# volivan239/raytracing-course-hw

Hardware: AMD Instinct MI355X
Metric: Msamples/sec at 1920x1080x256spp (higher is better)
Workload: dtype f32; 1 GPU; synth_room_v1_1920x1080x256; scene=synth_room_v1 (seed 20241223), triangles=268816, emissive_triangles=4204, width=1920, height=1080, spp=256, ray_depth=6, parallelism=pixel tiles 32x32 round-robin over 1 GPU(s), bvh_nodes=265605, bvh_depth=24, light_bvh_depth=19, device_bytes=120573816

## Files before the change

raytracing-course-hw_amd/csrc/device/rt_device.h:

```cpp
#pragma once
#include <hip/hip_runtime.h>
#include "rt_types.h"

#define RT_DEV __device__ __forceinline__

namespace rtamd {
namespace dev {

struct F3 { float x, y, z; };
RT_DEV F3 f3(float x, float y, float z) { F3 r; r.x = x; r.y = y; r.z = z; return r; }
RT_DEV F3 f3(const float *p) { return f3(p[0], p[1], p[2]); }
RT_DEV F3 operator+(F3 a, F3 b) { return f3(a.x + b.x, a.y + b.y, a.z + b.z); }
RT_DEV F3 operator-(F3 a, F3 b) { return f3(a.x - b.x, a.y - b.y, a.z - b.z); }
RT_DEV F3 operator*(F3 a, F3 b) { return f3(a.x * b.x, a.y * b.y, a.z * b.z); }
RT_DEV F3 operator*(float k, F3 p) { return f3(k * p.x, k * p.y, k * p.z); }
RT_DEV F3 neg(F3 a) { return f3(-a.x, -a.y, -a.z); }
RT_DEV float dot(F3 a, F3 b) { return a.x * b.x + a.y * b.y + a.z * b.z; }
RT_DEV F3 crossr(F3 a, F3 o) { return f3(a.z * o.y - a.y * o.z, a.x * o.z - a.z * o.x, a.y * o.x - a.x * o.y); }
RT_DEV float len2(F3 a) { return dot(a, a); }
RT_DEV float len(F3 a) { return sqrtf(len2(a)); }
RT_DEV F3 normalize(F3 a) { return (1.0f / len(a)) * a; }
RT_DEV float smin(float a, float b) { return (b < a) ? b : a; }
RT_DEV float smax(float a, float b) { return (a < b) ? b : a; }

// ... 193 lines not shown
    float yy = (c1 * T.a2 - c2 * T.a1) / T.den;
    float xx = T.a2 == 0 ? (c1 - T.b1 * yy) / T.a1 : (c2 - T.b2 * yy) / T.a2;
    u = xx; v = yy;
    if (u < 0 || v < 0 || u + v > 1) return false;
    return true;
}

RT_DEV bool tri_test_closer(const TriIsect &T, F3 o, F3 d, float keep_t, float &t, float &u, float &v, bool &inside) {
    F3 a = f3(T.ax, T.ay, T.az), n = f3(T.nx, T.ny, T.nz);
    F3 ro = o - a;
    float dn = dot(d, n);
    t = -dot(ro, n) / dn;
    if (!(t > 0 && t < RT_T_MAX)) return false;
    if (t > keep_t) return false;
    inside = dn > 0;
    F3 p = ro + t * d;
    float c1 = RT_MAGIC1_0 * p.x + RT_MAGIC1_1 * p.y + RT_MAGIC1_2 * p.z;
    float c2 = RT_MAGIC2_0 * p.x + RT_MAGIC2_1 * p.y + RT_MAGIC2_2 * p.z;
    float yy = (c1 * T.a2 - c2 * T.a1) / T.den;
    float xx = T.a2 == 0 ? (c1 - T.b1 * yy) / T.a1 : (c2 - T.b2 * yy) / T.a2;
    u = xx; v = yy;
    if (u < 0 || v < 0 || u + v > 1) return false;
    return true;
}

RT_DEV TriIsect load_isect(const TriIsect *p) {
    const float4 *q = reinterpret_cast<const float4 *>(p);
    float4 a = q[0], b = q[1], c = q[2];
    TriIsect T;
    T.ax = a.x; T.ay = a.y; T.az = a.z; T.nx = a.w;
    T.ny = b.x; T.nz = b.y; T.a1 = b.z; T.b1 = b.w;
    T.a2 = c.x; T.b2 = c.y; T.den = c.z; T.pad = __float_as_uint(c.w);
    return T;
}

struct RayInv { F3 o, inv; };
RT_DEV RayInv make_ray_inv(F3 o, F3 d) {
    RayInv r;
    r.o = o;
    float dx = fabsf(d.x) > 1e-30f ? d.x : copysignf(1e-30f, d.x);
    float dy = fabsf(d.y) > 1e-30f ? d.y : copysignf(1e-30f, d.y);
    float dz = fabsf(d.z) > 1e-30f ? d.z : copysignf(1e-30f, d.z);
    r.inv = f3(1.0f / dx, 1.0f / dy, 1.0f / dz);
    return r;
}
RT_DEV bool slab_test(float4 lo, float4 hi, const RayInv &r, float tbest, float &tnear) {
// ... 425 lines not shown
```

raytracing-course-hw_amd/csrc/device/rt_exact.h:

```cpp
#pragma once
#include "rt_kernels_hw8.h"

namespace rtamd {
namespace dev {

#define PT_SHADE_EXACT 4
#define WF_MISS 0xFFFFFFFFu
#define WF_INSIDE_BIT 0x40000000u
#define WF_GAP_SHIFT 24
#define WF_INDEX_MASK 0x00FFFFFFu
#define WF_SAMPLE_MASK 0x01FFFFFFu
#define WF_VERIFIED_BIT 0x80000000u

RT_DEV bool ref_box_test(F3 mn, F3 mx, F3 o, F3 d, float &t, bool &inside) {
    const F3 s = 0.5f * (mx - mn);
    const F3 oc = o - 0.5f * (mn + mx);
    const F3 a = neg(s) - oc, b = s - oc;
    const float a1x = a.x / d.x, a1y = a.y / d.y, a1z = a.z / d.z;
    const float a2x = b.x / d.x, a2y = b.y / d.y, a2z = b.z / d.z;
    const float t1x = smin(a1x, a2x), t2x = smax(a1x, a2x);
    const float t1y = smin(a1y, a2y), t2y = smax(a1y, a2y);
    const float t1z = smin(a1z, a2z), t2z = smax(a1z, a2z);
    const float t1 = smax(smax(t1x, t1y), t1z);
    const float t2 = smin(smin(t2x, t2y), t2z);
// ... 140 lines not shown
                const float4 mlo = rec[2 * m];
                if (slab_test(mlo, rec[2 * m + 1], r, RT_T_MAX, tn)) {
                    const uint32_t fi = __float_as_uint(mlo.w);
                    const TriIsect T = load_isect(S.tri_isect + fi);
                    float t, u, v; bool inside;
                    if (tri_test(T, o, d, t, u, v, inside)) {
                        const float4 *bx = reinterpret_cast<const float4 *>(S.tri_box) + 2 * (size_t)fi;
                        const float4 blo = bx[0], bhi = bx[1];
                        if (!pt_deep_inside(f3(blo.x, blo.y, blo.z), f3(bhi.x, bhi.y, bhi.z), o + t * d, d, t, S.box_c2)) pierced = true;
                    }
                }
            }
        }
    }
    return pierced;
}

RT_DEV bool pt_light_test(const LightRec *L, F3 x, F3 d, bool &last, uint32_t &index, float &t, float &u, float &v, bool &inside) {
    const TriIsect T = load_isect(&L->isect);
    last = (T.pad & 1u) != 0;
    index = T.pad >> 1;
    return tri_test(T, x, d, t, u, v, inside);
}
RT_DEV float pt_light_pdf_hit(const SceneView &S, const LightRec *L, F3 x, F3 d, float t, float u, float v, bool inside, bool &robust) {
    robust = true;
    const float4 *q = reinterpret_cast<const float4 *>(L) + 3;
    float4 q1 = q[1], q2 = q[2], q3 = q[3];
    float point_prob = q1.z;
    F3 n3 = f3(q1.w, q2.x, q2.y), dn1 = f3(q2.z, q2.w, q3.x), dn2 = f3(q3.y, q3.z, q3.w);
    F3 sn = n3 + u * dn1 + v * dn2;
    sn = normalize(sn);
    if (inside) sn = neg(sn);
    if (S.hw7) { const TriIsect T = load_isect(&L->isect); F3 n = f3(T.nx, T.ny, T.nz); sn = normalize(inside ? neg(n) : n); }
    F3 y = x + t * d;
    if (S.exact_boxes == 1u) {
        const float4 blo = q[4], bhi = q[5];
        robust = pt_box_robust(f3(blo.x, blo.y, blo.z), f3(bhi.x, bhi.y, bhi.z), y, d, t, S.box_c2);
    }
    return point_prob * len2(x - y) / fabsf(dot(d, sn));
}
RT_DEV float pt_light_pdf_one(const SceneView &S, const LightRec *L, F3 x, F3 d, bool &last, bool &robust, uint32_t &index) {
    TriIsect T = load_isect(&L->isect);
    last = (T.pad & 1u) != 0;
    index = T.pad >> 1;
    robust = true;
    float t, u, v; bool inside;
// ... 21 lines not shown
```

raytracing-course-hw_amd/csrc/device/rt_persistent.h:

```cpp
#pragma once
#include "rt_wavefront.h"

namespace rtamd {
namespace dev {

#define P8_WAVES 4
#define P8_THREADS (64 * P8_WAVES)
#define P8_PER_CU 5
#define PT_MAX_PATHS 5120
#define PT_MIN_GROUP 16
#define PT_NW (PT_MAX_PATHS / 32)
#define PT_BIT_T 1u
#define PT_BIT_L 2u
#define PT_NONE 0xFFFFFFFFu
#define PT_Q_TRACE 0
#define PT_Q_LIGHT 1
#define PT_Q_SHADE 2
#define PT_Q_XLIGHT 3
#define PT_Q_XTRACE 4
#define PT_N_LIVE 5
#define PT_W_TRACE 6
#define PT_W_LIGHT 7
#define PT_GSHIFT 15
#define PT_COST_TRACE_NODE 1u
// ... 87 lines not shown

struct PtParams {
    uint32_t n_groups;
    uint32_t group_shift;
    const uint32_t *group_ofs, *group_ids;
    uint32_t *group_cost;
    uint32_t resume;
    int refill, leaf_batch;
    int shade_min;
    int shade_thr0, shade_thr_step;
    int cost_t, cost_l;
    uint32_t front_first;
    int prio;
    unsigned long long deadline_ticks;
    unsigned long long *counters;
    unsigned long long *debug;
    float4 *trace_buf; uint32_t trace_cap; int32_t trace_pixel;
};

struct PtProf {
    unsigned long long t_role[5] = {0, 0, 0, 0, 0};
    unsigned long long iters[2] = {0, 0}, lane_iters[2] = {0, 0}, stints = 0, shade_batches = 0, shade_items = 0;
    unsigned long long t_part[2][3] = {{0, 0, 0}, {0, 0, 0}}, leaf_iters[2] = {0, 0}, leaf_lane_iters[2] = {0, 0}, light_hits = 0, light_tests = 0;
    unsigned long long t_sub[2][3] = {{0, 0, 0}, {0, 0, 0}}, refills[2] = {0, 0};
    unsigned long long light_reach[2] = {0, 0};
};
template <bool COUNT> struct PtLap {
    unsigned long long t;
    RT_DEV PtLap() : t(COUNT ? __builtin_amdgcn_s_memtime() : 0ull) {}
    RT_DEV void lap(unsigned long long &acc) { if (COUNT) { const unsigned long long n = __builtin_amdgcn_s_memtime(); acc += n - t; t = n; } }
};

struct PtWave {
    uint32_t nw, n_local, n_blocks, block;
    bool front_first;
    uint32_t cur[5];
};

template <class SH> RT_DEV uint32_t pt_gshift(const SH &sh) { return (uint32_t)__builtin_amdgcn_readfirstlane(__hip_atomic_load(&sh.cnt[PT_GSHIFT], __ATOMIC_RELAXED, __HIP_MEMORY_SCOPE_WORKGROUP)); }
template <class SH> RT_DEV uint32_t pt_slot(const SH &sh, uint32_t l) { const uint32_t g = pt_gshift(sh); return (sh.groups[l >> g] << g) | (l & ((1u << g) - 1u)); }
RT_DEV int pt_count(const int *p) { return __builtin_amdgcn_readfirstlane(__hip_atomic_load(p, __ATOMIC_RELAXED, __HIP_MEMORY_SCOPE_WORKGROUP)); }

RT_DEV int pt_leaf_batch(int leaf_batch, unsigned long long m_active) {
    const int cap = leaf_batch & 255, share = ((int)__popcll(m_active) * (leaf_batch >> 16) + 255) >> 8;
    return share < cap ? share : cap;
}
// ... 185 lines not shown
        clk.lap(prof.t_part[K][1]);
        const bool at_leaf = active && pend != RT_EMPTY_LEAF;
        if (COUNT) { prof.leaf_iters[K]++; prof.leaf_lane_iters[K] += __popcll(pt_ballot(at_leaf)); }
        if (at_leaf) {
            uint32_t i = pend & ~RT_LEAF_BIT, more = pend2, more2 = pend3;
            typename WK::Leaf lf;
            for (;;) {
                const bool last = w.test(i, sp, lf);
                if (COUNT) n_tris++;
                steps += WK::COST_TEST;
                if (!last) i++;
                else if (more == RT_EMPTY_LEAF) break;
                else { i = more & ~RT_LEAF_BIT; more = more2; more2 = RT_EMPTY_LEAF; }
            }
            const bool over = w.leaves_done(lf, sp);
            pend = RT_EMPTY_LEAF; pend2 = RT_EMPTY_LEAF; pend3 = RT_EMPTY_LEAF;
            if (cur == PT_DRAINED || over) end_walk();
        }
        clk.lap(prof.t_part[K][2]);
    }
}

template <class T> RT_DEV const T *pt_own_pointer(const T *p) { asm volatile("" : "+s"(p)); return p; }
struct PtTraceWalk {
    typedef PtTraceQueue Queue;
    static constexpr uint32_t COST_NODE = PT_COST_TRACE_NODE, COST_TEST = PT_COST_TRACE_TRI;
    const SceneView &S; const WfView &W; PtShared &sh; const PtParams &P; uint32_t (*stack)[64];
    const GpuNode4Q *nodes = pt_own_pointer(S.nodes4);
    const int lane = threadIdx.x & 63;
    F3 o = f3(0.f, 0.f, 0.f), d = f3(0.f, 0.f, 1.f);
    RayGrid ray = RT_GRID_RAY_IDLE;
    uint32_t hit = WF_MISS;
    float best_t = RT_T_MAX, best_u = 0.f, best_v = 0.f;
    float cull_t = RT_T_MAX, t2 = 2.f * RT_T_MAX, h_ray = 0.f;
    struct Leaf {};
    RT_DEV void begin(uint32_t slot) {
        const float4 *r = wf_rec(W, slot);
        float4 q0 = r[0], q1 = r[1];
        o = f3(q0.x, q0.y, q0.z); d = f3(q0.w, q1.x, q1.y);
        ray = make_ray_grid(S.grid, o, d);
        h_ray = S.exact_boxes ? pt_look_behind_abs(d, S.box_c2x) : 0.f;
        hit = WF_MISS; best_t = RT_T_MAX; cull_t = RT_T_MAX; t2 = 2.f * RT_T_MAX; best_u = 0.f; best_v = 0.f;
    }
    RT_DEV int step(uint32_t &cur, int &sp) { return pt_wide_step_nearest(nodes, ray, cull_t, stack, lane, sp, P8_STACK, cur); }
    RT_DEV void full() { best_t = PT_T_OVERFLOW; best_u = 0.f; best_v = 0.f; hit = 0u; t2 = PT_T_OVERFLOW; }
    RT_DEV bool test(uint32_t i, int, Leaf &) {
        TriIsect T = load_isect(S.tri_walk + i);
        float t, u, v; bool inside;
        const uint32_t fi = T.pad >> 1;
        if (tri_test_closer(T, o, d, cull_t, t, u, v, inside)) {
            const uint32_t best_i = hit & WF_INDEX_MASK;
            if (t < best_t || (t == best_t && fi < best_i)) {
                t2 = fminf(t2, best_t);
                best_t = t; best_u = u; best_v = v; hit = fi | (inside ? WF_INSIDE_BIT : 0u);
                cull_t = t + fmaxf(S.cull_k * t, h_ray);
            } else t2 = fminf(t2, t);
        }
        return (T.pad & 1u) != 0u;
    }
    RT_DEV bool leaves_done(Leaf &, int) { return false; }
    RT_DEV uint32_t end(uint32_t l, uint32_t slot, uint32_t steps) {
        wf_rec(W, slot)[2] = make_float4(best_t, best_u, best_v, __uint_as_float(S.exact_boxes && hit != WF_MISS ? hit | pt_gap_code(best_t, t2) : hit));
        pt_book_cost(sh, P, l, steps);
        return l;
    }
};

template <bool COUNT> struct PtLightWalk {
    typedef PtLightQueue<PT_Q_XLIGHT> Queue;
    static constexpr uint32_t COST_NODE = PT_COST_LIGHT_NODE, COST_TEST = PT_COST_LIGHT_TEST;
    const SceneView &S; const WfView &W; PtShared &sh; const PtParams &P; uint32_t (*stack)[64]; PtProf &prof;
    const GpuNode4Q *nodes = pt_own_pointer(S.light_walk_nodes4);
    const LightRec *lights = pt_own_pointer(S.lights_walk);
    const int lane = threadIdx.x & 63;
    bool overflow = false;
    int k = 0;
    F3 o = f3(0.f, 0.f, 0.f), d = f3(0.f, 0.f, 1.f);
    RayGrid ray = RT_GRID_RAY_IDLE;
    struct Leaf { bool held = false; uint32_t h_i = 0u, h_li = 0u; float h_t = 0.f, h_u = 0.f, h_v = 0.f; bool h_in = false; };
    RT_DEV void begin(uint32_t slot) {
        const float4 *r = wf_rec(W, slot);
        float4 q0 = r[0], q1 = r[1];
        o = f3(q0.x, q0.y, q0.z); d = f3(q0.w, q1.x, q1.y);
        ray = make_ray_grid(S.grid, o, d);
        k = 0; overflow = false;
    }
    RT_DEV int step(uint32_t &cur, int &sp) { return pt_wide_step_all(nodes, ray, stack, lane, sp, P8_STACK - 2 * k - 1, cur); }
    RT_DEV void full() { overflow = true; }
    RT_DEV void take(Leaf &lf, int sp) {
        bool robust;
        const float term = pt_light_pdf_hit(S, lights + lf.h_i, o, d, lf.h_t, lf.h_u, lf.h_v, lf.h_in, robust);
        if (COUNT && term != 0.f) prof.light_hits++;
        if (term != 0.f) {
            if (!robust || k >= WF_MAX_LIGHT_HITS || sp + 2 * k + 2 >= P8_STACK) overflow = true;
            else {
                int j = k;
                while (j > 0 && stack[P8_STACK - 1 - 2 * (j - 1)][lane] > lf.h_li) {
                    stack[P8_STACK - 1 - 2 * j][lane] = stack[P8_STACK - 1 - 2 * (j - 1)][lane];
                    stack[P8_STACK - 2 - 2 * j][lane] = stack[P8_STACK - 2 - 2 * (j - 1)][lane];
                    j--;
                }
                stack[P8_STACK - 1 - 2 * j][lane] = lf.h_li; stack[P8_STACK - 2 - 2 * j][lane] = __float_as_uint(term); k++;
            }
        }
        lf.held = false;
    }
    RT_DEV bool test(uint32_t i, int sp, Leaf &lf) {
        bool last, inside; uint32_t li; float t, u, v;
        if (COUNT) prof.light_tests++;
        if (pt_light_test(lights + i, o, d, last, li, t, u, v, inside)) {
            if (lf.held) take(lf, sp);
            lf.held = true; lf.h_i = i; lf.h_li = li; lf.h_t = t; lf.h_u = u; lf.h_v = v; lf.h_in = inside;
        }
        return last;
    }
    RT_DEV bool leaves_done(Leaf &lf, int sp) { if (lf.held) take(lf, sp); return false; }
    RT_DEV uint32_t end(uint32_t l, uint32_t slot, uint32_t steps) {
        pt_book_cost(sh, P, l, steps);
        if (overflow) return l | 0x80000000u;
        float v = 0.f;
        if (k == 1) v = __uint_as_float(stack[P8_STACK - 2][lane]);
        else if (k == 2) v = __uint_as_float(stack[P8_STACK - 2][lane]) + __uint_as_float(stack[P8_STACK - 4][lane]);
        else if (k > 2) {
            const uint32_t nl = S.n_lights;
            for (int j = 1; j < k; j++) {
                uint32_t a0 = stack[P8_STACK - 1 - 2 * (j - 1)][lane], b0 = stack[P8_STACK - 1 - 2 * j][lane];
                uint32_t len = b0 - a0;
                uint32_t lv = 31u - (uint32_t)__clz((int)len);
                uint16_t m0 = S.light_sep[(size_t)lv * nl + a0], m1 = S.light_sep[(size_t)lv * nl + (b0 - (1u << lv))];
                stack[j - 1][lane] = m0 < m1 ? m0 : m1;
            }
            for (int n = k; n > 1; n--) {
                int best = 1;
                uint32_t bd = stack[0][lane];
                for (int i = 2; i < n; i++) { uint32_t di = stack[i - 1][lane]; if (di > bd) { bd = di; best = i; } }
                float merged = __uint_as_float(stack[P8_STACK - 2 - 2 * (best - 1)][lane]) + __uint_as_float(stack[P8_STACK - 2 - 2 * best][lane]);
                stack[P8_STACK - 2 - 2 * (best - 1)][lane] = __float_as_uint(merged);
                for (int i = best; i < n - 1; i++) {
                    stack[P8_STACK - 2 - 2 * i][lane] = stack[P8_STACK - 2 - 2 * (i + 1)][lane];
// ... 293 lines not shown
            const uint32_t got = pt_pop(sh.need[PT_Q_SHADE], &sh.cnt[PT_Q_SHADE], wv.nw, wv.cur[PT_Q_SHADE], true, wv.front_first);
            __builtin_amdgcn_fence(__ATOMIC_ACQUIRE, "workgroup");
            if (pt_here(P.prio) == 2) __builtin_amdgcn_s_setprio(2);
            const PtShaded s = rl.shade(got, n_light, n_nodes, prof);
            __builtin_amdgcn_fence(__ATOMIC_RELEASE, "workgroup");
            if (s.trace || s.light) atomicOr(&sh.pending[got >> 4], ((s.trace ? PT_BIT_T : 0u) | (s.light ? PT_BIT_L : 0u)) << ((got & 15u) * 2u));
            pt_push(sh, PT_Q_TRACE, got, s.trace && !s.xtrace);
            pt_push(sh, PT_Q_LIGHT, got, s.light);
            pt_push(sh, PT_Q_XTRACE, got, s.xtrace);
            if (s.cost) atomicAdd(&sh.cost[got >> pt_gshift(sh)], s.cost);
            const unsigned long long done = pt_ballot(s.done);
            if (done && lane == 0) atomicSub(&sh.cnt[PT_N_LIVE], (int)__popcll(done));
            idle_spins = 0;
            if (pt_here(P.prio) == 2) __builtin_amdgcn_s_setprio(0);
            if (COUNT) { prof.shade_batches++; prof.shade_items += __popcll(pt_ballot(got != PT_NONE)); }
            clk.lap(prof.t_role[2]);
            continue;
        }
        if (nt + nl > 0) {
            const long long wt = (long long)nt * P.cost_t * (pt_count(&sh.cnt[PT_W_LIGHT]) + 1), wl = (long long)nl * P.cost_l * (pt_count(&sh.cnt[PT_W_TRACE]) + 1);
            if (pt_here(P.prio) == 1) __builtin_amdgcn_s_setprio(2);
            if (nl == 0 || (nt > 0 && wt >= wl)) {
                if (lane == 0) atomicAdd(&sh.cnt[PT_W_TRACE], 1);
                auto walk = rl.trace_walk();
                pt_walk_stint<RL::SLOTS, RL::DEFER, COUNT>(walk, sh, P, wv, stack, shade_thr, n_closest, n_nodes, n_tris, prof);
                if (lane == 0) atomicSub(&sh.cnt[PT_W_TRACE], 1);
                clk.lap(prof.t_role[0]);
            } else {
                if (lane == 0) atomicAdd(&sh.cnt[PT_W_LIGHT], 1);
                auto walk = rl.light_walk(prof);
                pt_walk_stint<RL::SLOTS, RL::DEFER, COUNT>(walk, sh, P, wv, stack, shade_thr, n_light, n_nodes, n_tris, prof);
                if (lane == 0) atomicSub(&sh.cnt[PT_W_LIGHT], 1);
                clk.lap(prof.t_role[1]);
            }
            if (pt_here(P.prio) == 1) __builtin_amdgcn_s_setprio(0);
            idle_spins = 0;
            if (COUNT) prof.stints++;
            continue;
        }
        if (pt_count(&sh.cnt[PT_N_LIVE]) <= 0) break;
        __builtin_amdgcn_s_sleep(8);
        clk.lap(prof.t_role[4]);
        if (++idle_spins > (1u << 24)) { gave_up = 2; break; }
    }
    if (gave_up && lane == 0 && P.counters) atomicAdd(&P.counters[gave_up == 1 ? CNT_DEADLINE : CNT_LOST_PATH], 1ull);
    pt_leave<RL::THREADS>(sh, P, wv);
    if (P.counters) {
        if (lane == 0 && n_closest) atomicAdd(&P.counters[CNT_CLOSEST], (unsigned long long)n_closest);
        if (lane == 0 && n_light) atomicAdd(&P.counters[CNT_LIGHT], (unsigned long long)n_light);
        if (COUNT) {
            atomicAdd(&P.counters[CNT_NODE_VISITS], n_nodes); atomicAdd(&P.counters[CNT_TRI_TESTS], n_tris);
            if (lane == 0) for (int i = 0; i < 5; i++) atomicAdd(&P.counters[CNT_ROLE_TIME + i], prof.t_role[i]);
        }
        rl.flush(lane, prof);
    }
    if (P.debug && lane == 0) atomicMax(&P.debug[3 * blockIdx.x + 1], __builtin_amdgcn_s_memrealtime());
}

template <bool COUNT_, int FEAT>
struct PtRoles {
    static constexpr bool COUNT = COUNT_;
    static constexpr int THREADS = P8_THREADS;
    static constexpr int SLOTS = 3;
    static constexpr bool DEFER = true;
    const SceneView &S; const RenderView &R; const WfView &W; PtShared &sh; const PtParams &P;
    uint32_t (*stack)[64] = sh.stack[__builtin_amdgcn_readfirstlane((int)(threadIdx.x >> 6))];
    uint32_t n_xtrace = 0, n_xlight = 0, n_discarded = 0;
    RT_DEV PtTraceWalk trace_walk() { return PtTraceWalk{S, W, sh, P, stack}; }
    RT_DEV PtLightWalk<COUNT> light_walk(PtProf &prof) { return PtLightWalk<COUNT>{S, W, sh, P, stack, prof}; }
    RT_DEV void seed(uint32_t slot, uint32_t gslot, int x, int y, Rng &rng, F3 sum) {
        if (R.sample_seeds) wf_sample_seed(R, rng, gslot, x, y, 0u);
        F3 o, d;
        wf_camera_ray(S, R, rng, x, y, o, d);
        float4 *r = wf_rec(W, slot);
        r[0] = make_float4(o.x, o.y, o.z, d.x);
        r[1] = make_float4(d.y, d.z, __uint_as_float(rng.x), rng.saved);
        r[2] = make_float4(0.f, 0.f, 0.f, 0.f);
        r[3] = make_float4(sum.x, sum.y, sum.z, __uint_as_float(wf_pack(0, rng.has_saved, R.accum ? (uint32_t)R.sample_first : 0u)));
    }
    RT_DEV uint32_t resumed_sample(uint32_t slot) { return (__float_as_uint(reinterpret_cast<const float *>(wf_rec(W, slot) + 3)[3]) >> 6) & WF_SAMPLE_MASK; }
    RT_DEV bool seed_wire(uint32_t slot) {
        if (!S.n_tripwire_groups) return false;
        const float4 *nr = wf_rec(W, slot);
        const float4 n0 = nr[0], n1 = nr[1];
        return pt_tripwire(S, f3(n0.x, n0.y, n0.z), f3(n0.w, n1.x, n1.y));
    }
    RT_DEV bool rare(PtWave &wv) {
        const bool queued = pt_count(&sh.cnt[PT_Q_XLIGHT]) + pt_count(&sh.cnt[PT_Q_XTRACE]) > 0;
        if (queued) pt_exact_batch(S, W, sh, wv, &stack[0][0], n_xlight, n_xtrace);
        return queued;
    }
// ... 31 lines not shown
                    float *pdf = reinterpret_cast<float *>(wf_entry(W, pt_slot(sh, got), depth)) + 3;
                    *pdf = *pdf + 0.f / S.n_lights_f;
                }
            }
        }
        n_light += __popcll(pt_ballot(settled));
        if (COUNT && settled) n_nodes += (unsigned long long)settle_steps;
        PtShaded s;
        s.trace = next;
        s.light = with_light && !settled;
        s.xtrace = (got != PT_NONE && todo == PT_SHADE_EXACT) || wire;
        s.done = got != PT_NONE && (todo == 0 || todo == WF_PARKED);
        if (got != PT_NONE && todo != PT_SHADE_EXACT) s.cost = (uint32_t)PT_COST_SHADE + (settled ? PT_COST_LIGHT_NODE * (uint32_t)settle_steps : 0u);
        return s;
    }
    RT_DEV void flush(uint32_t lane, const PtProf &prof) {
        if (lane == 0) {
            if (n_discarded) atomicAdd(&P.counters[CNT_DISCARDED], (unsigned long long)n_discarded);
            if (n_xtrace) atomicAdd(&P.counters[CNT_EXACT_CLOSEST], (unsigned long long)n_xtrace);
            if (n_xlight) atomicAdd(&P.counters[CNT_EXACT_LIGHT], (unsigned long long)n_xlight);
        }
        if (!COUNT) return;
        atomicAdd(&P.counters[CNT_P8_LIGHT_HITS], prof.light_hits); atomicAdd(&P.counters[CNT_P8_LIGHT_TESTS], prof.light_tests);
        atomicAdd(&P.counters[CNT_P8_LIGHT_REACH], prof.light_reach[0]); atomicAdd(&P.counters[CNT_P8_LIGHT_REACH + 1], prof.light_reach[1]);
        if (lane == 0) {
            atomicAdd(&P.counters[CNT_P8_WALK_ITERS], prof.iters[0]); atomicAdd(&P.counters[CNT_P8_WALK_ITERS + 1], prof.lane_iters[0]);
            atomicAdd(&P.counters[CNT_P8_WALK_ITERS + 2], prof.iters[1]); atomicAdd(&P.counters[CNT_P8_WALK_ITERS + 3], prof.lane_iters[1]);
            atomicAdd(&P.counters[CNT_P8_STINTS], prof.stints); atomicAdd(&P.counters[CNT_P8_SHADE_BATCHES], prof.shade_batches); atomicAdd(&P.counters[CNT_P8_SHADE_ITEMS], prof.shade_items);
            for (int k = 0; k < 3; k++) atomicAdd(&P.counters[CNT_P8_HANDOFF_TIME + k], prof.t_sub[0][k]);
            atomicAdd(&P.counters[CNT_P8_HANDOFFS], prof.refills[0]);
            for (int w = 0; w < 2; w++) {
                for (int k = 0; k < 3; k++) atomicAdd(&P.counters[CNT_P8_WALK_TIME + 3 * w + k], prof.t_part[w][k]);
                atomicAdd(&P.counters[CNT_P8_LEAF_ITERS + 2 * w], prof.leaf_iters[w]); atomicAdd(&P.counters[CNT_P8_LEAF_ITERS + 2 * w + 1], prof.leaf_lane_iters[w]);
            }
        }
    }
};

template <bool COUNT, int FEAT>
__global__ __launch_bounds__(P8_THREADS, P8_PER_CU) void pt_persistent_kernel(SceneView S, RenderView R, WfView W, PtParams P) {
    __shared__ PtShared sh;
    PtRoles<COUNT, FEAT> roles{S, R, W, sh, P};
    pt_run(roles);
}

}
// ... 2 lines not shown
```

raytracing-course-hw_amd/csrc/device/rt_persistent_hw6.h:

```cpp
#pragma once
#include "rt_persistent.h"
#include "rt_kernels_hw6.h"
#include "rt_exact.h"

namespace rtamd {
namespace dev {

#define P6_WAVES 4
#define P6_THREADS (64 * P6_WAVES)
#define P6_PER_CU 5
#define P6_MAX_PATHS 2304
#define P6_NW (P6_MAX_PATHS / 32)
#define P6_XBATCH 8
#define P6_SLICE_WORDS (P6_STACK * 64 / P6_XBATCH)
#define P6_COST_TRACE_STEP 1u
#define P6_COST_LIGHT_STEP 2u
#define P6_COST_SHADE 10u
#define P6_LIGHT_PRETEST false
#define P6_MERGE_HITS 13
#define P6_Q_SLOW 3
#define P6_REC 56u
#define P6_PENDING 32u
#define P6_LIGHT_ONLY 64u
#define P6_VERIFIED 128u
// ... 614 lines not shown
        const F3 xo = f3(q0.x, q0.y, q0.z), xd = f3(q0.w, q1.x, q1.y);
        if (S.n_tris < (1u << 18)  && p6_all_hits(S, xo, xd, xstack, xhits, xk)) { p6_sort_hits(xhits, xk); ref_closest_hit6_along(S, xo, xd, xhits, xk, xstack, bt, bin, bhit); }
        else ref_closest_hit6(S, xo, xd, xstack, bt, bin, bhit);
        r[2] = make_float4(bt, __uint_as_float(bhit), __uint_as_float(bin ? 1u : 0u), 0.f);
        float *pk = reinterpret_cast<float *>(r + 3) + 3;
        *pk = __uint_as_float(__float_as_uint(*pk) | P6_VERIFIED);
    }
    n_exact += __popcll(pt_ballot(got != PT_NONE));
    __builtin_amdgcn_fence(__ATOMIC_RELEASE, "workgroup");
    pt_push(sh, PT_Q_SHADE, got, got != PT_NONE);
}
static_assert(sizeof(P6Shared) <= 25 * 1280, "five workgroups per CU: 25 LDS granules of 1,280 bytes each");
static_assert(RT6_STACK_SIZE + P6_XHITS <= P6_SLICE_WORDS && 6 * RT6_MAX_LIGHT_HITS <= P6_SLICE_WORDS, "the rare roles' work arrays must fit a slice of the wave's stack area");

template <bool COUNT_>
struct P6Roles {
    static constexpr bool COUNT = COUNT_;
    static constexpr int THREADS = P6_THREADS;
    static constexpr int SLOTS = 2;
    static constexpr bool DEFER = false;
    const SceneView6 &S; const RenderView &R; const W6View &W; P6Shared &sh; const PtParams &P;
    uint32_t (*stack)[64] = sh.stack[__builtin_amdgcn_readfirstlane((int)(threadIdx.x >> 6))];
    uint32_t n_slow = 0, n_exact = 0, n_xlight = 0;
    RT_DEV P6TraceWalk trace_walk() { return P6TraceWalk{S, W, sh, P, stack}; }
    RT_DEV P6LightWalk light_walk(PtProf &) { return P6LightWalk{S, W, sh, P, stack}; }
    RT_DEV void seed(uint32_t slot, uint32_t, int x, int y, Rng &rng, F3 sum) {
        F3 o, d;
        p6_camera_ray(S, R, rng, x, y, o, d);
        float4 *r = p6_rec(W, slot);
        r[0] = make_float4(o.x, o.y, o.z, d.x);
        r[1] = make_float4(d.y, d.z, __uint_as_float(rng.x), rng.saved);
        r[2] = make_float4(0.f, 0.f, 0.f, 0.f);
        r[3] = make_float4(sum.x, sum.y, sum.z, __uint_as_float(p6_pack(0, rng.has_saved, R.accum ? (uint32_t)R.sample_first : 0u, 0u)));
    }
    RT_DEV uint32_t resumed_sample(uint32_t slot) { return __float_as_uint(reinterpret_cast<const float *>(p6_rec(W, slot) + 3)[3]) >> 8; }
    RT_DEV bool seed_wire(uint32_t) { return false; }
    RT_DEV bool rare(PtWave &wv) {
        const bool slow = pt_count(&sh.cnt[P6_Q_SLOW]) > 0, exact = !slow && pt_count(&sh.cnt[P6_Q_XTRACE]) > 0;
        if (slow) {
            const uint32_t got = pt_pop(sh.need[P6_Q_SLOW], &sh.cnt[P6_Q_SLOW], wv.nw, wv.cur[P6_Q_SLOW], true);
            __builtin_amdgcn_fence(__ATOMIC_ACQUIRE, "workgroup");
            bool batch = false;
            if (got != PT_NONE) {
                float4 *r = p6_rec(W, pt_slot(sh, got));
                const uint32_t kw = reinterpret_cast<const uint32_t *>(r + 7)[0];
                if (COUNT && P.counters) atomicAdd(&P.counters[CNT_P6_SLOW_HITS + ((kw & 0x7FFFFFFFu) < 15u ? (kw & 0x7FFFFFFFu) : 15u)], 1ull);
                if ((kw >> 31) || kw > (uint32_t)P6_MERGE_HITS) batch = true;
// ... 38 lines not shown
```

raytracing-course-hw_amd/csrc/device/rt_types.h:

```cpp
#pragma once
#include <stdint.h>

namespace rtamd {

#define RT_MAX_DEPTH 16
#define RT_STACK_SIZE 64
#define P8_STACK 24

enum CounterSlot {
    CNT_CLOSEST = 0,
    CNT_LIGHT = 1,
    CNT_NODE_VISITS = 2,
    CNT_TRI_TESTS = 3,
    CNT_WF_NODE_ITERS = 4,
    CNT_WF_LEAF_PHASES = 5,
    CNT_WF_LEAF_LANES = 6,
    CNT_WF_REFILLS = 7,
    CNT_WF_LANE_NODES = 8,
    CNT_WF_LANE_TRIS = 9,
    CNT_DISCARDED = 10,
    CNT_WF_SLOW_LIGHT = 11,
    CNT_P6_EXACT_LIGHT = 11,
    CNT_EXACT_CLOSEST = 12,
    CNT_EXACT_LIGHT = 13,
    CNT_P6_SLOW_LIGHT = 13,
    CNT_LOST_PATH = 14,
    CNT_WANT_HISTOGRAMS = 15,
    CNT_WF_HIST_CLOSEST = 16,
    CNT_ROLE_TIME = 16,
    CNT_P8_WALK_ITERS = 21,
    CNT_P8_STINTS = 25,
    CNT_P8_SHADE_BATCHES = 26,
    CNT_P8_SHADE_ITEMS = 27,
    CNT_DEADLINE = 29,
    CNT_P8_LIGHT_REACH = 30,
    CNT_WF_HIST_LIGHT = 32,
    CNT_P6_SLOW_HITS = 32,
    CNT_P8_WALK_TIME = 48,
    CNT_P8_LEAF_ITERS = 54,
    CNT_P8_LIGHT_HITS = 58,
    CNT_P8_LIGHT_TESTS = 59,
    CNT_P8_HANDOFF_TIME = 60,
    CNT_P8_HANDOFFS = 63,
    CNT_SLOTS = 64
};
#define CNT_BYTES (CNT_SLOTS * sizeof(unsigned long long))

struct GpuNode {
    float lo0[3]; int32_t child0;
    float hi0[3]; int32_t cnt0;
    float lo1[3]; int32_t child1;
    float hi1[3]; int32_t cnt1;
};
static_assert(sizeof(GpuNode) == 64, "GpuNode must be 64 bytes");

struct GpuNode4Q { uint32_t rec[4][4]; };
static_assert(sizeof(GpuNode4Q) == 64, "GpuNode4Q must be 64 bytes");
#define RT_GRID_CELLS 65000.0
#define RT_GRID_BORDER 4
struct NodeGrid { float lo[3], step[3], istep[3]; };
// ... 111 lines not shown
```

raytracing-course-hw_amd/csrc/rtamd_api.hip:

```cpp
#include <hip/hip_runtime.h>
#include <algorithm>
#include <cmath>
#include <cstdio>
#include <cstring>
#include <functional>
#include <memory>
#include <string>
#include <vector>
#include "../../include/rtamd.h"
#include "host/knobs.h"
#include "host/rt_scene.h"
#include "host/rt_accum_state.h"
#include "device/rt_kernels_hw8.h"
#include "device/rt_wavefront.h"
#include "device/rt_persistent.h"
#include "device/rt_kernels_hw6.h"
#include "device/rt_persistent_hw6.h"
#include "device/rt_kernels_txt.h"
#include "device/rt_kernels_hw2.h"
#include "device/rt_kernels_hw4.h"
#include "device/rt_kernels_hw5.h"

using namespace rtamd;

// ... 409 lines not shown
            for (int b = 0; b < 16; b++) fprintf(stderr, " %llu", h_cnt[CNT_P6_SLOW_HITS + b]);
            fprintf(stderr, "\n");
            fprintf(stderr, "[rtamd] persistent hw6 kernel, wave time by role: closest-hit walks %.1f %%, light walks %.1f %%, shading %.1f %%, slow light sums %.1f %%, idle %.1f %%\n",
                    100 * role[0] / tt, 100 * role[1] / tt, 100 * role[2] / tt, 100 * role[3] / tt, 100 * role[4] / tt);
        }
    } else if (times && count) {
        const unsigned long long *iters = h_cnt + CNT_P8_WALK_ITERS, n_light = h_cnt[CNT_LIGHT];
        fprintf(stderr, "[rtamd] persistent kernel, wave time by role: closest-hit walks %.1f %%, light walks %.1f %%, shading %.1f %%, exact walks %.2f %%, idle %.1f %%; "
                        "walker lane utilisation: closest hit %.1f of 64 (%llu wave iterations), light %.1f of 64 (%llu); %llu stints, %llu shade batches of %.1f paths\n",
                100 * role[0] / tt, 100 * role[1] / tt, 100 * role[2] / tt, 100 * role[3] / tt, 100 * role[4] / tt,
                (double)iters[1] / nz(iters[0]), iters[0], (double)iters[3] / nz(iters[2]), iters[2],
                h_cnt[CNT_P8_STINTS], h_cnt[CNT_P8_SHADE_BATCHES], (double)h_cnt[CNT_P8_SHADE_ITEMS] / nz(h_cnt[CNT_P8_SHADE_BATCHES]));
        for (int w = 0; w < 2; w++) {
            const unsigned long long *part = h_cnt + CNT_P8_WALK_TIME + 3 * w, *leaf = h_cnt + CNT_P8_LEAF_ITERS + 2 * w;
            const double tw = (double)(part[0] + part[1] + part[2]);
            fprintf(stderr, "[rtamd]   %s walker's wave time: hand-off and refill %.1f %%, inner nodes %.1f %%, leaves %.1f %%; leaf passes %llu with %.1f of 64 lanes\n",
                    w ? "light" : "closest-hit", 100 * part[0] / tw, 100 * part[1] / tw, 100 * part[2] / tw, leaf[0], (double)leaf[1] / nz(leaf[0]));
        }
        const unsigned long long *handoff = h_cnt + CNT_P8_HANDOFF_TIME, tests = h_cnt[CNT_P8_LIGHT_TESTS], hits = h_cnt[CNT_P8_LIGHT_HITS], *reach = h_cnt + CNT_P8_LIGHT_REACH;
        fprintf(stderr, "[rtamd]   closest-hit walker's hand-off points: %llu; of their time: publishing finished walks %.1f %%, taking new ones from the bitmap %.1f %%, reading their rays %.1f %% (the rest: the test itself)\n",
                h_cnt[CNT_P8_HANDOFFS], 100.0 * handoff[0] / nz(h_cnt[CNT_P8_WALK_TIME]), 100.0 * handoff[1] / nz(h_cnt[CNT_P8_WALK_TIME]), 100.0 * handoff[2] / nz(h_cnt[CNT_P8_WALK_TIME]));
        fprintf(stderr, "[rtamd]   light tests %llu (%.2f per light sum), hits %llu (%.2f per light sum); triangle tests of closest-hit walks %llu (%.2f per query)\n",
                tests, (double)tests / nz(n_light), hits, (double)hits / nz(n_light), h_cnt[CNT_TRI_TESTS] - tests, (double)(h_cnt[CNT_TRI_TESTS] - tests) / nz(h_cnt[CNT_CLOSEST]));
        fprintf(stderr, "[rtamd]   light sums whose walk ends at the light tree's root %llu (%.1f %%), one level below it %llu (%.1f %%); settled by the shader: level %d\n",
                reach[0], 100.0 * reach[0] / nz(n_light), reach[1], 100.0 * reach[1] / nz(n_light), PT_LIGHT_SETTLE);
    }
    if (!times) return;
    std::vector<unsigned long long> dbg((size_t)scene->pt_blocks * 3);
    HIP_CHECK(hipMemcpy(dbg.data(), scene->d_pt_debug, dbg.size() * sizeof(unsigned long long), hipMemcpyDeviceToHost));
    unsigned long long t0 = ~0ull, tmin = ~0ull, tmax = 0; double tsum = 0;
    for (uint32_t b = 0; b < scene->pt_blocks; b++) if (dbg[3 * b] && dbg[3 * b] < t0) t0 = dbg[3 * b];
    for (uint32_t b = 0; b < scene->pt_blocks; b++) { unsigned long long e = dbg[3 * b + 1] - t0; tmin = e < tmin ? e : tmin; tmax = e > tmax ? e : tmax; tsum += (double)e; }
    if (const char *dump = env_str("RTAMD_DUMP_WG")) {
        if (FILE *f = fopen(dump, "w")) {
            for (uint32_t b = 0; b < scene->pt_blocks; b++) fprintf(f, "%u %.4f %.4f %llu\n", b, (dbg[3 * b] - t0) * 1e-5, (dbg[3 * b + 1] - t0) * 1e-5, dbg[3 * b + 2]);
            fclose(f);
        }
    }
    if (!hw6)
        fprintf(stderr, "[rtamd] persistent pipeline: %u launches; re-deal of the sub-tiles took %.2f ms on the host (slowest workgroup / mean under the round-robin deal: %.3f)\n",
                scene->pt_launches, scene->pt_rebalance_ms, scene->pt_imbalance);
    fprintf(stderr, "[rtamd] %s (last launch): %u workgroups, exit times min / mean / max = %.3f / %.3f / %.3f ms after the first start",
            kernel, scene->pt_blocks, tmin * 1e-5, tsum / scene->pt_blocks * 1e-5, tmax * 1e-5);
    if (!hw6) fprintf(stderr, "; exact closest hits %llu, exact light sums %llu of %llu + %llu queries", h_cnt[CNT_EXACT_CLOSEST], h_cnt[CNT_EXACT_LIGHT], h_cnt[CNT_CLOSEST], h_cnt[CNT_LIGHT]);
    fprintf(stderr, "\n");
}
// ... 447 lines not shown
```

Measured before the change: 480.3 Msamples/s.

## Add conservative division-free triangle prefilter and defer exact leaf tests

Adds a conservative triangle rejection filter that uses hardware reciprocal approximations plus error bounds in place of exact divisions. Both the closest-hit and light walkers now run this cheap filter per leaf triangle, hold at most one surviving candidate, and run the exact test only on survivors when the next one appears or the leaf ends. The aim is to cut divisions and divergent exact-test work in leaf loops. The cost is reloading triangle data for survivors, some extra arithmetic, and reliance on the error bound being conservative enough to keep results exact; profiling counters are added too.

Result: slower. 471.4 Msamples/s (-1.9%).

```diff
diff --git a/raytracing-course-hw_amd/csrc/device/rt_device.h b/raytracing-course-hw_amd/csrc/device/rt_device.h
--- a/raytracing-course-hw_amd/csrc/device/rt_device.h
+++ b/raytracing-course-hw_amd/csrc/device/rt_device.h
@@ -239,6 +239,36 @@
     u = xx; v = yy;
     if (u < 0 || v < 0 || u + v > 1) return false;
     return true;
+}
+
+#define RT_FILTER_K 8.0f
+RT_DEV bool tri_filter(const TriIsect &T, F3 o, F3 d, float keep_t) {
+    const float U4 = 0x1p-21f;
+    F3 a = f3(T.ax, T.ay, T.az), n = f3(T.nx, T.ny, T.nz);
+    F3 ro = o - a;
+    float dn = dot(d, n);
+    float nn = -dot(ro, n);
+    const float tq = nn * __builtin_amdgcn_rcpf(dn);
+    const bool behind = tq < 0;
+    const bool regular = __builtin_amdgcn_classf(tq, 0x100);
+    const bool far = tq > fminf(keep_t, RT_T_MAX) * (1.f + 0x1p-20f);
+    const float px = __builtin_fmaf(tq, d.x, ro.x), py = __builtin_fmaf(tq, d.y, ro.y), pz = __builtin_fmaf(tq, d.z, ro.z);
+    const float c1 = __builtin_fmaf(RT_MAGIC1_2, pz, __builtin_fmaf(RT_MAGIC1_1, py, RT_MAGIC1_0 * px));
+    const float c2 = __builtin_fmaf(RT_MAGIC2_2, pz, __builtin_fmaf(RT_MAGIC2_1, py, RT_MAGIC2_0 * px));
+    const float rd = __builtin_amdgcn_rcpf(T.den);
+    const float yy = __builtin_fmaf(c1, T.a2, -(c2 * T.a1)) * rd;
+    const bool first = T.a2 == 0;
+    const float A = first ? T.a1 : T.a2, B = first ? T.b1 : T.b2, C = first ? c1 : c2;
+    const float ra = __builtin_amdgcn_rcpf(A);
+    const float By = B * yy;
+    const float xx = (C - By) * ra;
+    const float S = __builtin_fmaf(fabsf(tq), fabsf(d.x) + fabsf(d.y) + fabsf(d.z), fabsf(ro.x) + fabsf(ro.y) + fabsf(ro.z));
+    const float Ec = (RT_FILTER_K * 0x1p-23f) * S;
+    const float Ey = __builtin_fmaf(Ec * (fabsf(T.a1) + fabsf(T.a2)), fabsf(rd), U4 * fabsf(yy));
+    const float Ex = __builtin_fmaf(__builtin_fmaf(U4, fabsf(C) + fabsf(By), __builtin_fmaf(fabsf(B), Ey, Ec)), fabsf(ra), U4 * fabsf(xx));
+    const bool outside = (yy < -Ey) | (xx < -Ex) | (xx + yy > (Ex + Ey) + (1.f + U4));
+    const bool bounded = regular & __builtin_amdgcn_classf(rd, 0x108) & __builtin_amdgcn_classf(ra, 0x108);
+    return !(behind | (regular & far) | (bounded & outside));
 }
 
 RT_DEV TriIsect load_isect(const TriIsect *p) {
diff --git a/raytracing-course-hw_amd/csrc/device/rt_exact.h b/raytracing-course-hw_amd/csrc/device/rt_exact.h
--- a/raytracing-course-hw_amd/csrc/device/rt_exact.h
+++ b/raytracing-course-hw_amd/csrc/device/rt_exact.h
@@ -186,6 +186,11 @@
     index = T.pad >> 1;
     return tri_test(T, x, d, t, u, v, inside);
 }
+RT_DEV bool pt_light_filter(const LightRec *L, F3 x, F3 d, bool &last) {
+    const TriIsect T = load_isect(&L->isect);
+    last = (T.pad & 1u) != 0;
+    return tri_filter(T, x, d, RT_T_MAX);
+}
 RT_DEV float pt_light_pdf_hit(const SceneView &S, const LightRec *L, F3 x, F3 d, float t, float u, float v, bool inside, bool &robust) {
     robust = true;
     const float4 *q = reinterpret_cast<const float4 *>(L) + 3;
diff --git a/raytracing-course-hw_amd/csrc/device/rt_persistent.h b/raytracing-course-hw_amd/csrc/device/rt_persistent.h
--- a/raytracing-course-hw_amd/csrc/device/rt_persistent.h
+++ b/raytracing-course-hw_amd/csrc/device/rt_persistent.h
@@ -133,6 +133,8 @@
     unsigned long long t_role[5] = {0, 0, 0, 0, 0};
     unsigned long long iters[2] = {0, 0}, lane_iters[2] = {0, 0}, stints = 0, shade_batches = 0, shade_items = 0;
     unsigned long long t_part[2][3] = {{0, 0, 0}, {0, 0, 0}}, leaf_iters[2] = {0, 0}, leaf_lane_iters[2] = {0, 0}, light_hits = 0, light_tests = 0;
+    unsigned long long trace_survivors = 0, light_survivors = 0;
+    unsigned long long loop_settles[2] = {0, 0};
     unsigned long long t_sub[2][3] = {{0, 0, 0}, {0, 0, 0}}, refills[2] = {0, 0};
     unsigned long long light_reach[2] = {0, 0};
 };
@@ -364,10 +366,11 @@
 }
 
 template <class T> RT_DEV const T *pt_own_pointer(const T *p) { asm volatile("" : "+s"(p)); return p; }
-struct PtTraceWalk {
+#define PT_NOT_HELD 0xFFFFFFFFu
+template <bool COUNT> struct PtTraceWalk {
     typedef PtTraceQueue Queue;
     static constexpr uint32_t COST_NODE = PT_COST_TRACE_NODE, COST_TEST = PT_COST_TRACE_TRI;
-    const SceneView &S; const WfView &W; PtShared &sh; const PtParams &P; uint32_t (*stack)[64];
+    const SceneView &S; const WfView &W; PtShared &sh; const PtParams &P; uint32_t (*stack)[64]; PtProf &prof;
     const GpuNode4Q *nodes = pt_own_pointer(S.nodes4);
     const int lane = threadIdx.x & 63;
     F3 o = f3(0.f, 0.f, 0.f), d = f3(0.f, 0.f, 1.f);
@@ -375,7 +378,7 @@
     uint32_t hit = WF_MISS;
     float best_t = RT_T_MAX, best_u = 0.f, best_v = 0.f;
     float cull_t = RT_T_MAX, t2 = 2.f * RT_T_MAX, h_ray = 0.f;
-    struct Leaf {};
+    struct Leaf { uint32_t held = PT_NOT_HELD; };
     RT_DEV void begin(uint32_t slot) {
         const float4 *r = wf_rec(W, slot);
         float4 q0 = r[0], q1 = r[1];
@@ -386,8 +389,9 @@
     }
     RT_DEV int step(uint32_t &cur, int &sp) { return pt_wide_step_nearest(nodes, ray, cull_t, stack, lane, sp, P8_STACK, cur); }
     RT_DEV void full() { best_t = PT_T_OVERFLOW; best_u = 0.f; best_v = 0.f; hit = 0u; t2 = PT_T_OVERFLOW; }
-    RT_DEV bool test(uint32_t i, int, Leaf &) {
-        TriIsect T = load_isect(S.tri_walk + i);
+    RT_DEV void settle(Leaf &lf) {
+        TriIsect T = load_isect(S.tri_walk + lf.held);
+        lf.held = PT_NOT_HELD;
         float t, u, v; bool inside;
         const uint32_t fi = T.pad >> 1;
         if (tri_test_closer(T, o, d, cull_t, t, u, v, inside)) {
@@ -398,9 +402,17 @@
                 cull_t = t + fmaxf(S.cull_k * t, h_ray);
             } else t2 = fminf(t2, t);
         }
+    }
+    RT_DEV bool test(uint32_t i, int, Leaf &lf) {
+        TriIsect T = load_isect(S.tri_walk + i);
+        if (tri_filter(T, o, d, cull_t)) {
+            if (COUNT) prof.trace_survivors++;
+            if (lf.held != PT_NOT_HELD) { if (COUNT) prof.loop_settles[0]++; settle(lf); }
+            lf.held = i;
+        }
         return (T.pad & 1u) != 0u;
     }
-    RT_DEV bool leaves_done(Leaf &, int) { return false; }
+    RT_DEV bool leaves_done(Leaf &lf, int) { if (lf.held != PT_NOT_HELD) settle(lf); return false; }
     RT_DEV uint32_t end(uint32_t l, uint32_t slot, uint32_t steps) {
         wf_rec(W, slot)[2] = make_float4(best_t, best_u, best_v, __uint_as_float(S.exact_boxes && hit != WF_MISS ? hit | pt_gap_code(best_t, t2) : hit));
         pt_book_cost(sh, P, l, steps);
@@ -419,7 +431,7 @@
     int k = 0;
     F3 o = f3(0.f, 0.f, 0.f), d = f3(0.f, 0.f, 1.f);
     RayGrid ray = RT_GRID_RAY_IDLE;
-    struct Leaf { bool held = false; uint32_t h_i = 0u, h_li = 0u; float h_t = 0.f, h_u = 0.f, h_v = 0.f; bool h_in = false; };
+    struct Leaf { uint32_t held = PT_NOT_HELD; };
     RT_DEV void begin(uint32_t slot) {
         const float4 *r = wf_rec(W, slot);
         float4 q0 = r[0], q1 = r[1];
@@ -430,33 +442,35 @@
     RT_DEV int step(uint32_t &cur, int &sp) { return pt_wide_step_all(nodes, ray, stack, lane, sp, P8_STACK - 2 * k - 1, cur); }
     RT_DEV void full() { overflow = true; }
     RT_DEV void take(Leaf &lf, int sp) {
-        bool robust;
-        const float term = pt_light_pdf_hit(S, lights + lf.h_i, o, d, lf.h_t, lf.h_u, lf.h_v, lf.h_in, robust);
+        const LightRec *L = lights + lf.held;
+        lf.held = PT_NOT_HELD;
+        bool last, inside, robust = true; uint32_t h_li; float t, u, v;
+        const float term = pt_light_test(L, o, d, last, h_li, t, u, v, inside) ? pt_light_pdf_hit(S, L, o, d, t, u, v, inside, robust) : 0.f;
         if (COUNT && term != 0.f) prof.light_hits++;
         if (term != 0.f) {
             if (!robust || k >= WF_MAX_LIGHT_HITS || sp + 2 * k + 2 >= P8_STACK) overflow = true;
             else {
                 int j = k;
-                while (j > 0 && stack[P8_STACK - 1 - 2 * (j - 1)][lane] > lf.h_li) {
+                while (j > 0 && stack[P8_STACK - 1 - 2 * (j - 1)][lane] > h_li) {
                     stack[P8_STACK - 1 - 2 * j][lane] = stack[P8_STACK - 1 - 2 * (j - 1)][lane];
                     stack[P8_STACK - 2 - 2 * j][lane] = stack[P8_STACK - 2 - 2 * (j - 1)][lane];
                     j--;
                 }
-                stack[P8_STACK - 1 - 2 * j][lane] = lf.h_li; stack[P8_STACK - 2 - 2 * j][lane] = __float_as_uint(term); k++;
-            }
-        }
-        lf.held = false;
+                stack[P8_STACK - 1 - 2 * j][lane] = h_li; stack[P8_STACK - 2 - 2 * j][lane] = __float_as_uint(term); k++;
+            }
+        }
     }
     RT_DEV bool test(uint32_t i, int sp, Leaf &lf) {
-        bool last, inside; uint32_t li; float t, u, v;
+        bool last;
         if (COUNT) prof.light_tests++;
-        if (pt_light_test(lights + i, o, d, last, li, t, u, v, inside)) {
-            if (lf.held) take(lf, sp);
-            lf.held = true; lf.h_i = i; lf.h_li = li; lf.h_t = t; lf.h_u = u; lf.h_v = v; lf.h_in = inside;
+        if (pt_light_filter(lights + i, o, d, last)) {
+            if (COUNT) prof.light_survivors++;
+            if (lf.held != PT_NOT_HELD) { if (COUNT) prof.loop_settles[1]++; take(lf, sp); }
+            lf.held = i;
         }
         return last;
     }
-    RT_DEV bool leaves_done(Leaf &lf, int sp) { if (lf.held) take(lf, sp); return false; }
+    RT_DEV bool leaves_done(Leaf &lf, int sp) { if (lf.held != PT_NOT_HELD) take(lf, sp); return false; }
     RT_DEV uint32_t end(uint32_t l, uint32_t slot, uint32_t steps) {
         pt_book_cost(sh, P, l, steps);
         if (overflow) return l | 0x80000000u;
@@ -796,7 +810,7 @@
             if (pt_here(P.prio) == 1) __builtin_amdgcn_s_setprio(2);
             if (nl == 0 || (nt > 0 && wt >= wl)) {
                 if (lane == 0) atomicAdd(&sh.cnt[PT_W_TRACE], 1);
-                auto walk = rl.trace_walk();
+                auto walk = rl.trace_walk(prof);
                 pt_walk_stint<RL::SLOTS, RL::DEFER, COUNT>(walk, sh, P, wv, stack, shade_thr, n_closest, n_nodes, n_tris, prof);
                 if (lane == 0) atomicSub(&sh.cnt[PT_W_TRACE], 1);
                 clk.lap(prof.t_role[0]);
@@ -840,7 +854,7 @@
     const SceneView &S; const RenderView &R; const WfView &W; PtShared &sh; const PtParams &P;
     uint32_t (*stack)[64] = sh.stack[__builtin_amdgcn_readfirstlane((int)(threadIdx.x >> 6))];
     uint32_t n_xtrace = 0, n_xlight = 0, n_discarded = 0;
-    RT_DEV PtTraceWalk trace_walk() { return PtTraceWalk{S, W, sh, P, stack}; }
+    RT_DEV PtTraceWalk<COUNT> trace_walk(PtProf &prof) { return PtTraceWalk<COUNT>{S, W, sh, P, stack, prof}; }
     RT_DEV PtLightWalk<COUNT> light_walk(PtProf &prof) { return PtLightWalk<COUNT>{S, W, sh, P, stack, prof}; }
     RT_DEV void seed(uint32_t slot, uint32_t gslot, int x, int y, Rng &rng, F3 sum) {
         if (R.sample_seeds) wf_sample_seed(R, rng, gslot, x, y, 0u);
@@ -918,6 +932,8 @@
         }
         if (!COUNT) return;
         atomicAdd(&P.counters[CNT_P8_LIGHT_HITS], prof.light_hits); atomicAdd(&P.counters[CNT_P8_LIGHT_TESTS], prof.light_tests);
+        atomicAdd(&P.counters[CNT_P8_TRACE_SURVIVORS], prof.trace_survivors); atomicAdd(&P.counters[CNT_P8_LIGHT_SURVIVORS], prof.light_survivors);
+        atomicAdd(&P.counters[CNT_P8_LOOP_SETTLES], prof.loop_settles[0]); atomicAdd(&P.counters[CNT_P8_LOOP_SETTLES + 1], prof.loop_settles[1]);
         atomicAdd(&P.counters[CNT_P8_LIGHT_REACH], prof.light_reach[0]); atomicAdd(&P.counters[CNT_P8_LIGHT_REACH + 1], prof.light_reach[1]);
         if (lane == 0) {
             atomicAdd(&P.counters[CNT_P8_WALK_ITERS], prof.iters[0]); atomicAdd(&P.counters[CNT_P8_WALK_ITERS + 1], prof.lane_iters[0]);
diff --git a/raytracing-course-hw_amd/csrc/device/rt_persistent_hw6.h b/raytracing-course-hw_amd/csrc/device/rt_persistent_hw6.h
--- a/raytracing-course-hw_amd/csrc/device/rt_persistent_hw6.h
+++ b/raytracing-course-hw_amd/csrc/device/rt_persistent_hw6.h
@@ -660,7 +660,7 @@
     const SceneView6 &S; const RenderView &R; const W6View &W; P6Shared &sh; const PtParams &P;
     uint32_t (*stack)[64] = sh.stack[__builtin_amdgcn_readfirstlane((int)(threadIdx.x >> 6))];
     uint32_t n_slow = 0, n_exact = 0, n_xlight = 0;
-    RT_DEV P6TraceWalk trace_walk() { return P6TraceWalk{S, W, sh, P, stack}; }
+    RT_DEV P6TraceWalk trace_walk(PtProf &) { return P6TraceWalk{S, W, sh, P, stack}; }
     RT_DEV P6LightWalk light_walk(PtProf &) { return P6LightWalk{S, W, sh, P, stack}; }
     RT_DEV void seed(uint32_t slot, uint32_t, int x, int y, Rng &rng, F3 sum) {
         F3 o, d;
diff --git a/raytracing-course-hw_amd/csrc/device/rt_types.h b/raytracing-course-hw_amd/csrc/device/rt_types.h
--- a/raytracing-course-hw_amd/csrc/device/rt_types.h
+++ b/raytracing-course-hw_amd/csrc/device/rt_types.h
@@ -36,6 +36,9 @@
     CNT_P8_LIGHT_REACH = 30,
     CNT_WF_HIST_LIGHT = 32,
     CNT_P6_SLOW_HITS = 32,
+    CNT_P8_TRACE_SURVIVORS = 32,
+    CNT_P8_LIGHT_SURVIVORS = 33,
+    CNT_P8_LOOP_SETTLES = 34,
     CNT_P8_WALK_TIME = 48,
     CNT_P8_LEAF_ITERS = 54,
     CNT_P8_LIGHT_HITS = 58,
diff --git a/raytracing-course-hw_amd/csrc/rtamd_api.hip b/raytracing-course-hw_amd/csrc/rtamd_api.hip
--- a/raytracing-course-hw_amd/csrc/rtamd_api.hip
+++ b/raytracing-course-hw_amd/csrc/rtamd_api.hip
@@ -455,6 +455,9 @@
                 h_cnt[CNT_P8_HANDOFFS], 100.0 * handoff[0] / nz(h_cnt[CNT_P8_WALK_TIME]), 100.0 * handoff[1] / nz(h_cnt[CNT_P8_WALK_TIME]), 100.0 * handoff[2] / nz(h_cnt[CNT_P8_WALK_TIME]));
         fprintf(stderr, "[rtamd]   light tests %llu (%.2f per light sum), hits %llu (%.2f per light sum); triangle tests of closest-hit walks %llu (%.2f per query)\n",
                 tests, (double)tests / nz(n_light), hits, (double)hits / nz(n_light), h_cnt[CNT_TRI_TESTS] - tests, (double)(h_cnt[CNT_TRI_TESTS] - tests) / nz(h_cnt[CNT_CLOSEST]));
+        const unsigned long long kept_l = h_cnt[CNT_P8_LIGHT_SURVIVORS], kept_t = h_cnt[CNT_P8_TRACE_SURVIVORS];
+        fprintf(stderr, "[rtamd]   leaf filter: %llu of the light tests survive (%.1f %%, %.2f per hit; %llu settled inside the loop), %llu of the triangle tests (%.1f %%, %.2f per closest-hit query; %llu settled inside the loop)\n",
+                kept_l, 100.0 * kept_l / nz(tests), (double)kept_l / nz(hits), h_cnt[CNT_P8_LOOP_SETTLES + 1], kept_t, 100.0 * kept_t / nz(h_cnt[CNT_TRI_TESTS] - tests), (double)kept_t / nz(h_cnt[CNT_CLOSEST]), h_cnt[CNT_P8_LOOP_SETTLES]);
         fprintf(stderr, "[rtamd]   light sums whose walk ends at the light tree's root %llu (%.1f %%), one level below it %llu (%.1f %%); settled by the shader: level %d\n",
                 reach[0], 100.0 * reach[0] / nz(n_light), reach[1], 100.0 * reach[1] / nz(n_light), PT_LIGHT_SETTLE);
     }
```
